# wvangansbeke/LaneDetection_End2End

Hardware: AMD Instinct MI355X
Metric: images/sec fwd+bwd, 256x512 2-lane bs32 (higher is better)
Workload: dtype f32; 1 GPU; BEV ERFNet + fused WLS fit + Area loss, 2 lanes, 256x512, batch 32 per GPU, fp32, train mode (BN batch stats, Dropout2d on), fwd+bwd, optimizer excluded; global_batch=32, parallelism=dp1, grad_allreduce=none

## Files before the change

lanedetection_end2end_amd/csrc/lf_conv.hip:

```cpp
#include <stdlib.h>
#include <string.h>

#include <atomic>
#include <map>
#include <mutex>
#include <tuple>
#include <utility>

#include <hip/hip_ext.h>

#include "lf_conv.h"
#include "lf_ldsdma.h"
#include "lf_types.h"

typedef float f32x4 __attribute__((ext_vector_type(4)));

namespace {

constexpr int MT = 4;
constexpr int WG_WAVES = 4;
constexpr int PIX_PER_WG = WG_WAVES * MT * 16;

__device__ __forceinline__ f32x4 ldg4(const float* p) { return *reinterpret_cast<const f32x4*>(p); }
typedef unsigned u32x4v __attribute__((vector_size(16)));
__device__ __forceinline__ __amdgpu_buffer_rsrc_t make_rsrc(const void* base, unsigned bytes) {
    return __builtin_amdgcn_make_buffer_rsrc(const_cast<void*>(base), 0, bytes, 0x00020000);
}
__device__ __forceinline__ f32x4 ldb4(__amdgpu_buffer_rsrc_t r, unsigned voff, unsigned soff) {
    return __builtin_bit_cast(f32x4, __builtin_amdgcn_raw_buffer_load_b128(r, (int)voff, (int)soff, 0));
}
__device__ __forceinline__ f32x4 zero4() { f32x4 z = {0.f, 0.f, 0.f, 0.f}; return z; }
typedef int i32x4 __attribute__((ext_vector_type(4)));
__device__ __forceinline__ f32x4 max0(f32x4 v) {
    i32x4 b = __builtin_bit_cast(i32x4, v);
    b.x = b.x > 0 ? b.x : 0; b.y = b.y > 0 ? b.y : 0; b.z = b.z > 0 ? b.z : 0; b.w = b.w > 0 ? b.w : 0;
    return __builtin_bit_cast(f32x4, b);
}
__device__ __forceinline__ f32x4 relu_keep_nan(f32x4 v) {
    v.x = v.x <= 0.f ? 0.f : v.x; v.y = v.y <= 0.f ? 0.f : v.y; v.z = v.z <= 0.f ? 0.f : v.z; v.w = v.w <= 0.f ? 0.f : v.w;
    return v;
}
__device__ __forceinline__ f32x4 keep_pos(f32x4 v, f32x4 m) {
    v.x = m.x > 0.f ? v.x : 0.f; v.y = m.y > 0.f ? v.y : 0.f; v.z = m.z > 0.f ? v.z : 0.f; v.w = m.w > 0.f ? v.w : 0.f;
    return v;
}
typedef unsigned u32x2v __attribute__((vector_size(8)));
template <bool S16>
__device__ __forceinline__ f32x4 epi_ld(__amdgpu_buffer_rsrc_t r, unsigned off, unsigned soff = 0u) {
    if constexpr (S16) {
        const u32x2v q = __builtin_amdgcn_raw_buffer_load_b64(r, (int)(off * 2u), (int)(soff * 2u), 0);
        f32x4 v;
        v.x = __uint_as_float(q[0] << 16); v.y = __uint_as_float(q[0] & 0xffff0000u);
        v.z = __uint_as_float(q[1] << 16); v.w = __uint_as_float(q[1] & 0xffff0000u);
        return v;
    } else return ldb4(r, off * 4u, soff * 4u);
}
template <bool S16>
__device__ __forceinline__ void epi_st(__amdgpu_buffer_rsrc_t r, unsigned off, f32x4 v) {
    if constexpr (S16) {
        lf_bf16x4 b;
        b[0] = (lf_bf16)v.x; b[1] = (lf_bf16)v.y; b[2] = (lf_bf16)v.z; b[3] = (lf_bf16)v.w;
        __builtin_amdgcn_raw_buffer_store_b64(__builtin_bit_cast(u32x2v, b), r, (int)(off * 2u), 0, 0);
    } else __builtin_amdgcn_raw_buffer_store_b128(__builtin_bit_cast(u32x4v, v), r, (int)(off * 4u), 0, 0);
}
__device__ __forceinline__ f32x4 round_bf16(f32x4 v) {
    v.x = (float)(lf_bf16)v.x; v.y = (float)(lf_bf16)v.y; v.z = (float)(lf_bf16)v.z; v.w = (float)(lf_bf16)v.w;
    return v;
}
typedef float f32x2 __attribute__((ext_vector_type(2)));
typedef __bf16 bf16x2 __attribute__((ext_vector_type(2)));
__device__ __forceinline__ unsigned split_pair(f32x2& v) {
    const unsigned u = __builtin_bit_cast(unsigned, __builtin_convertvector(v, bf16x2));
    v.x -= __uint_as_float(u << 16);
    v.y -= __uint_as_float(u & 0xffff0000u);
    return u;
}
template <int CTRL>
__device__ __forceinline__ float dpp_mov(float v) {
    return __builtin_bit_cast(float, __builtin_amdgcn_update_dpp(0, __builtin_bit_cast(int, v), CTRL, 0xf, 0xf, false));
}
__device__ __forceinline__ f32x4 bcast16(f32x4 v) {
    f32x4 r;
    r.x = dpp_mov<0x150>(v.x); r.y = dpp_mov<0x150>(v.y); r.z = dpp_mov<0x150>(v.z); r.w = dpp_mov<0x150>(v.w);
    return r;
}
__device__ __forceinline__ float sum16(float v) {
    v += dpp_mov<0xB1>(v);
    v += dpp_mov<0x4E>(v);
    v += dpp_mov<0x124>(v);
    v += dpp_mov<0x128>(v);
    return v;
}

#define LF_EPI_GROUPS 1
#define LF_EPI_ONE_TILE false
#define LF_EPI_TID threadIdx.x
#define LF_EPI_ROW1 false
#define LF_EPI_PIVOT true
#define LF_EPI_ACC(n, m) acc[n][m]
#define LF_EPI_FIRST(m) ((m) == 0)
#define LF_EPI_ROW_OK(tg) true
#define LF_EPI_HEAD \
      \
    const bool stats = (epi & (LF_EPI_STATS_SQ | LF_EPI_STATS_XHAT)) != 0; \
    constexpr bool NOBIAS = EPIC >= 0 && !(EPIC & LF_EPI_BIAS) && (EPIC & (LF_EPI_MASK | LF_EPI_ADD | LF_EPI_MASKBN | LF_EPI_STATS_XHAT)) != 0; \
    constexpr int NC = (NT % 2 == 0 && !LF_EPI_ONE_TILE) ? 2 : 1; \
     \
    constexpr bool HOISTM = HOISTV && !(EPIC >= 0 && (EPIC & LF_EPI_MASKBN) && (EPIC & LF_EPI_STATS_XHAT)); \
    const __amdgpu_buffer_rsrc_t r_dst = make_rsrc(a.dst, 0xffffffffu), r_add = make_rsrc(a.add_src, 0xffffffffu), \
                                 r_msk = make_rsrc(a.mask_src, 0xffffffffu), r_aux = make_rsrc(a.aux, 0xffffffffu), \
                                 r_bias = make_rsrc(a.bias, 0xffffffffu), r_msc = make_rsrc(a.msc, 0xffffffffu), \
                                 r_msh = make_rsrc(a.msh, 0xffffffffu), r_dm = make_rsrc(a.dm, 0xffffffffu); \
     \
    f32x4 s1[NT], s2[NT], bs[NOBIAS ? 1 : NT], hv[HOISTV ? NT : 1][2], piv[LF_EPI_PIVOT ? NT : 1]; \
_Pragma("unroll") \
    for (int n = 0; n < NT; ++n) { \
        const int co = cob + n * 16 + kq * 4; \
        s1[n] = zero4(); s2[n] = zero4(); piv[LF_EPI_PIVOT ? n : 0] = zero4(); \
        if constexpr (!NOBIAS) bs[n] = a.bias ? ldb4(r_bias, co * 4u, 0u) : zero4(); \
        if (HOISTV) { \
            if (HOISTM && (epi & LF_EPI_MASKBN)) { hv[n][0] = ldb4(r_msc, co * 4u, 0u); hv[n][1] = ldb4(r_msh, co * 4u, 0u); } \
        } \
    }
#define LF_EPI_TILE(m) \
    { \
        const unsigned dbase = (unsigned)(((pn[m] * g.Hd + pi[m] * g.dsh + g.dah) * g.Wd + pj[m] * g.dsw + g.daw) * g.d_pix + g.d_choff + cob + kq * 4); \
_Pragma("unroll") \
        for (int n0 = 0; n0 < NT; n0 += NC) { \
        f32x4 la[NC], lm[NC], lx[NC], ld[NC]; \
_Pragma("unroll") \
        for (int j = 0; j < NC; ++j) { \
            const int n = n0 + j; \
            if (epi & LF_EPI_ADD) la[j] = epi_ld<S16>(r_add, dbase + n * 16); \
            if (epi & LF_EPI_MASK) lm[j] = epi_ld<S16>(r_msk, dbase + n * 16); \
            if (epi & (LF_EPI_MASKBN | LF_EPI_STATS_XHAT)) lx[j] = epi_ld<S16>(r_aux, dbase + n * 16); \
            if ((epi & LF_EPI_STATS_XHAT) && a.dm && !LF_EPI_ROW1) ld[j] = ldb4(r_dm, (unsigned)(pn[m] * g.Cd + cob + n * 16 + kq * 4) * 4u, 0u); \
        } \
_Pragma("unroll") \
        for (int j = 0; j < NC; ++j) { \
            const int n = n0 + j; \
            f32x4 v = LF_EPI_ACC(n, m); \
            if constexpr (!NOBIAS) v += bs[n]; \
            if (epi & LF_EPI_ADD) v += la[j]; \
            if (epi & LF_EPI_MASK) v = keep_pos(v, lm[j]); \
            const int co = cob + n * 16 + kq * 4;    \
            if (epi & LF_EPI_MASKBN) v = keep_pos(v, lx[j] * (HOISTM ? hv[HOISTV ? n : 0][0] : ldb4(r_msc, co * 4u, 0u)) + (HOISTM ? hv[HOISTV ? n : 0][1] : ldb4(r_msh, co * 4u, 0u))); \
            if (epi & LF_EPI_RELU) v = S16 ? relu_keep_nan(v) : max0(v); \
            if (S16) v = round_bf16(v);    \
            if (pv[m]) epi_st<S16>(r_dst, dbase + n * 16, v); \
            if (!pv[m]) v = zero4(); \
            if (epi & LF_EPI_STATS_SQ) { \
                if (LF_EPI_PIVOT && LF_EPI_FIRST(m)) piv[LF_EPI_PIVOT ? n : 0] = bcast16(v); \
                f32x4 dv = LF_EPI_PIVOT ? v - piv[LF_EPI_PIVOT ? n : 0] : v; \
                if (!pv[m]) dv = zero4(); \
                s1[n] += dv; s2[n] += dv * dv; \
            } \
            if (epi & LF_EPI_STATS_XHAT) { \
                const f32x4 gm = (a.dm && !LF_EPI_ROW1) ? v * ld[j] : v; \
                s1[n] += gm; s2[n] += gm * lx[j];       \
            } \
        } \
        } \
    }
#define LF_EPI_TAIL \
    if (LF_EPI_ROW1 && (epi & LF_EPI_STATS_XHAT) && a.dm) { \
         \
_Pragma("unroll") \
        for (int n = 0; n < NT; ++n) { \
            const f32x4 dmv = ldb4(r_dm, (unsigned)(pn[0] * g.Cd + cob + n * 16 + kq * 4) * 4u, 0u); \
            s1[n] *= dmv; s2[n] *= dmv; \
        } \
    } \
    if (stats) { \
         \
        const int EW = wave & 3, EG = wave >> 2; \
        __shared__ float sred[LF_EPI_GROUPS][WG_WAVES][NT][4][8]; \
_Pragma("unroll") \
        for (int n = 0; n < NT; ++n) { \
            f32x4 r1, r2; \
            r1.x = sum16(s1[n].x); r1.y = sum16(s1[n].y); r1.z = sum16(s1[n].z); r1.w = sum16(s1[n].w); \
            r2.x = sum16(s2[n].x); r2.y = sum16(s2[n].y); r2.z = sum16(s2[n].z); r2.w = sum16(s2[n].w); \
            if (epi & LF_EPI_STATS_SQ) {       \
                const unsigned lf_t0 = (bx * (unsigned)(WG_WAVES * LF_EPI_GROUPS) + (unsigned)wave) * 64u; \
                const float nw = lf_t0 < npix ? (float)min(npix - lf_t0, 64u) : 0.f; \
                const float rn = nw > 0.f ? 1.f / nw : 0.f; \
                r2 = r2 - r1 * r1 * rn; \
                r2.x = fmaxf(r2.x, 0.f); r2.y = fmaxf(r2.y, 0.f); r2.z = fmaxf(r2.z, 0.f); r2.w = fmaxf(r2.w, 0.f); \
                if (LF_EPI_PIVOT) r1 = r1 + piv[LF_EPI_PIVOT ? n : 0] * nw; \
            } \
            if (pl == 0) { \
                float* d = sred[EG][EW][n][kq]; \
                d[0] = r1.x; d[1] = r1.y; d[2] = r1.z; d[3] = r1.w; d[4] = r2.x; d[5] = r2.y; d[6] = r2.z; d[7] = r2.w; \
            } \
        } \
        __syncthreads(); \
        if ((LF_EPI_TID & 255) < NT * 4 * 8 && LF_EPI_ROW_OK(LF_EPI_TID >> 8)) { \
            const int tg = LF_EPI_TID >> 8, tt = LF_EPI_TID & 255; \
            const int j = tt & 7, q = (tt >> 3) & 3, n = tt >> 5; \
            float v = sred[tg][0][n][q][j] + sred[tg][1][n][q][j] + sred[tg][2][n][q][j] + sred[tg][3][n][q][j]; \
            if ((epi & LF_EPI_STATS_SQ) && j >= 4) {       \
                const unsigned lf_tb = (bx * (unsigned)LF_EPI_GROUPS + (unsigned)tg) * (unsigned)(WG_WAVES * 64); \
                float nwv[4], sw[4], nt = 0.f, st = 0.f; \
_Pragma("unroll") \
                for (int w = 0; w < 4; ++w) { \
                    const unsigned t0w = lf_tb + (unsigned)w * 64u; \
                    nwv[w] = t0w < npix ? (float)min(npix - t0w, 64u) : 0.f; \
                    sw[w] = sred[tg][w][n][q][j - 4]; \
                    nt += nwv[w]; st += sw[w]; \
                } \
                const float mg = nt > 0.f ? st / nt : 0.f; \
_Pragma("unroll") \
                for (int w = 0; w < 4; ++w) \
                    if (nwv[w] > 0.f) { const float dmw = sw[w] / nwv[w] - mg; v += nwv[w] * dmw * dmw; } \
            } \
            const int co = cob + n * 16 + q * 4 + (j & 3); \
            a.stats[((long)(j >> 2) * g.Cd + co) * a.stats_ld + ((long)bx * LF_EPI_GROUPS + tg)] = v;       \
        } \
    }
#define LF_TAPGEMM_EPILOGUE \
    __builtin_amdgcn_s_setprio(3);    \
    LF_EPI_HEAD \
_Pragma("unroll") \
    for (int m = 0; m < MT; ++m) LF_EPI_TILE(m) \
    LF_EPI_TAIL

extern __shared__ __attribute__((aligned(16))) unsigned char lf_tap_lds[];
constexpr size_t LF_TAP_LDS_PER_TAP = (size_t)WG_WAVES * 64 * (sizeof(uint4) + sizeof(unsigned));

template <int NT, int PROC, int EPIC = -1, bool ROW1 = false, bool DBG = false>
__global__ __launch_bounds__(256, (EPIC >= 0 || NT < 4) ? 2 : 1) void tapgemm_kernel(const LfTapGeom g, const LfTapArgs a, const int pro, const int epi_rt) {
    const int epi = EPIC >= 0 ? EPIC : epi_rt;
    constexpr bool S16 = false, HOISTV = EPIC >= 0;
    unsigned long long tstamp[4] = {0ull, 0ull, 0ull, 0ull};
    if constexpr (DBG) tstamp[0] = __builtin_amdgcn_s_memrealtime();
    const unsigned npix = (unsigned)(g.N * g.Hl * g.Wl);
    const int cob = blockIdx.y * NT * 16;
    const unsigned ntiles = (npix + PIX_PER_WG - 1) / PIX_PER_WG;
    unsigned t_first = blockIdx.x, t_stride = gridDim.x, t_end = ntiles;
    if ((gridDim.x & 7u) == 0 && (ntiles & 7u) == 0) {
        const unsigned per = ntiles >> 3;
        t_first = (blockIdx.x & 7u) * per + (blockIdx.x >> 3); t_stride = gridDim.x >> 3; t_end = (blockIdx.x & 7u) * per + per;
    }
    for (unsigned bx = t_first; bx < t_end; bx += t_stride) {
    unsigned tid = threadIdx.x;
    asm volatile("" : "+v"(tid));
    const int lane = tid & 63, wave = tid >> 6;
    const int pl = lane & 15, kq = lane >> 4;
    const unsigned tile0 = (bx * WG_WAVES + (ROW1 ? __builtin_amdgcn_readfirstlane(wave) : wave)) * (MT * 16);

    int pn[MT], pi[MT], pj[MT];
    bool pv[MT];
    if constexpr (ROW1) {
        const unsigned q = tile0 < npix ? tile0 : 0u;
        const unsigned r = q / (unsigned)g.Wl;
        const int j0 = __builtin_amdgcn_readfirstlane((int)(q - r * (unsigned)g.Wl));
        const int n0 = __builtin_amdgcn_readfirstlane((int)(r / (unsigned)g.Hl));
        const int i0 = __builtin_amdgcn_readfirstlane((int)r) - n0 * g.Hl;
#pragma unroll
        for (int m = 0; m < MT; ++m) { pv[m] = tile0 < npix; pn[m] = n0; pi[m] = i0; pj[m] = j0 + m * 16 + pl; }
// ... 103 lines not shown
        if constexpr (DBG) tstamp[1] = __builtin_amdgcn_s_memrealtime();
        Step A, B;
        issue(A);
        finish(A);
        const int npairs = (nsteps + 1) >> 1;
        for (int pr = 0; pr < npairs; ++pr) {
            mma_restart(A);
            __builtin_amdgcn_sched_barrier(0);
            issue(B);
            __builtin_amdgcn_sched_barrier(0);
            mma(A, 1); mma(A, 2);
            __builtin_amdgcn_sched_barrier(0);
            finish(B);
            mma(A, 3);
            __builtin_amdgcn_sched_barrier(0);
            mma(B, 0);
            __builtin_amdgcn_sched_barrier(0);
            issue(A);
            __builtin_amdgcn_sched_barrier(0);
            mma(B, 1); mma(B, 2);
            __builtin_amdgcn_sched_barrier(0);
            finish(A);
            mma(B, 3);
            __builtin_amdgcn_sched_barrier(0);
        }
    }

#pragma unroll
    for (int n = 0; n < NT; ++n)
#pragma unroll
        for (int m = 0; m < MT; ++m) acc[n][m] += accl[n][m];
    if constexpr (!ROW1) {
        unsigned tid2 = threadIdx.x;
        asm volatile("" : "+v"(tid2));
        const unsigned tile0b = (bx * WG_WAVES + (tid2 >> 6)) * (MT * 16);
#pragma unroll
        for (int m = 0; m < MT; ++m) {
            const unsigned p = tile0b + m * 16 + (tid2 & 15u);
            pv[m] = p < npix;
            const unsigned q = pv[m] ? p : 0u;
            const unsigned r = q / (unsigned)g.Wl;
            pj[m] = (int)(q - r * (unsigned)g.Wl);
            pn[m] = (int)(r / (unsigned)g.Hl);
            pi[m] = (int)(r - (unsigned)pn[m] * (unsigned)g.Hl);
        }
    }
    if constexpr (DBG) {
        asm volatile("" ::"v"(acc[0][0][0]));
        tstamp[2] = __builtin_amdgcn_s_memrealtime();
    }
#undef LF_EPI_ONE_TILE
#define LF_EPI_ONE_TILE (!ROW1 && EPIC == (LF_EPI_ADD | LF_EPI_MASK | LF_EPI_STATS_XHAT))
#undef LF_EPI_TID
#define LF_EPI_TID tid
#undef LF_EPI_ROW1
#define LF_EPI_ROW1 ROW1
    LF_TAPGEMM_EPILOGUE
#undef LF_EPI_ONE_TILE
#define LF_EPI_ONE_TILE false
#undef LF_EPI_TID
#define LF_EPI_TID threadIdx.x
#undef LF_EPI_ROW1
#define LF_EPI_ROW1 false
    if (stats && bx + t_stride < t_end) __syncthreads();
    __builtin_amdgcn_s_setprio(0);
    }
    if constexpr (DBG) {
        asm volatile("s_waitcnt vmcnt(0)" ::: "memory");
        tstamp[3] = __builtin_amdgcn_s_memrealtime();
        const int lane = threadIdx.x & 63, wave = threadIdx.x >> 6;
        if (lane == 0 && a.dbg) {
            unsigned long long* d = a.dbg + ((unsigned long long)(blockIdx.y * gridDim.x + blockIdx.x) * WG_WAVES + wave) * 8;
            d[0] = tstamp[0]; d[1] = tstamp[1]; d[2] = tstamp[2]; d[3] = tstamp[3];
            unsigned hwid, xcc;
            asm volatile("s_getreg_b32 %0, hwreg(HW_REG_HW_ID)" : "=s"(hwid));
            asm volatile("s_getreg_b32 %0, hwreg(HW_REG_XCC_ID)" : "=s"(xcc));
            d[4] = (unsigned long long)hwid | ((unsigned long long)xcc << 32);
        }
    }
}

template <int CS, int PROC, int EPIC, int G>
__global__ __launch_bounds__(256 * G, G == 1 ? 2 : 1) void tapstream_kernel(const LfTapGeom g, const LfTapArgs a) {
    constexpr int NT = 4, NCG = CS / 16, NS = 3 * NCG, R = 8;
    constexpr int epi = EPIC;
    constexpr bool S16 = false, HOISTV = true;
    static_assert((4 * NS) % R == 0 && R <= NS && NS % 2 == 0, "ring positions and K-step pairs must be compile-time");
    const unsigned npix = (unsigned)(g.N * g.Hl * g.Wl);
    const int cob = blockIdx.y * 64;
    const unsigned ntiles = (npix + PIX_PER_WG - 1) / PIX_PER_WG, nunits = (ntiles + G - 1) / G;
    unsigned u_first = blockIdx.x, u_stride = gridDim.x, u_end = nunits;
    if ((gridDim.x & 7u) == 0 && (nunits & 7u) == 0) {
        const unsigned per = nunits >> 3;
        u_first = (blockIdx.x & 7u) * per + (blockIdx.x >> 3); u_stride = gridDim.x >> 3; u_end = (blockIdx.x & 7u) * per + per;
    }
    const int lane = threadIdx.x & 63, wave = threadIdx.x >> 6;
    const int pl = lane & 15, kq = lane >> 4;
    const unsigned wtile = (unsigned)__builtin_amdgcn_readfirstlane(wave);


    f32x4* const wl = reinterpret_cast<f32x4*>(lf_tap_lds);
    float* const pvec = reinterpret_cast<float*>(wl + NS * 256);
    struct WT { int n0, i0, j0; bool v; };
    auto coords = [&](unsigned u, bool live) -> WT {
        const unsigned tile0 = (u * (unsigned)(4 * G) + wtile) * 64u;
        WT c;
        c.v = live && tile0 < npix;
        const unsigned q = c.v ? tile0 : 0u;
        const unsigned r = q / (unsigned)g.Wl;
        c.j0 = __builtin_amdgcn_readfirstlane((int)(q - r * (unsigned)g.Wl));
        c.n0 = __builtin_amdgcn_readfirstlane((int)(r / (unsigned)g.Hl));
        c.i0 = __builtin_amdgcn_readfirstlane((int)r) - c.n0 * g.Hl;
        return c;
    };
    auto xoff = [&](const WT& c, int sub, int t, bool& in) -> unsigned {
        const int sy = c.i0 * g.ssh + g.tdh[t], sx = (c.j0 + sub * 16 + pl) * g.ssw + g.tdw[t];
        in = c.v && sy >= 0 && sy < g.Hs && sx >= 0 && sx < g.Ws;
        const int syc = min(max(sy, 0), g.Hs - 1), sxc = min(max(sx, 0), g.Ws - 1);
        const unsigned o = (unsigned)(((c.n0 * g.Hs + syc) * g.Ws + sxc) * g.s_pix + g.s_choff + kq * 4) * 4u;
        return (PROC == 0 && !in) ? LF_OOB : o;
    };
    const __amdgpu_buffer_rsrc_t rx = make_rsrc(a.src, (unsigned)min((long)g.N * g.Hs * g.Ws * g.s_pix * 4, (long)LF_OOB));
    auto xload = [&](const WT& c, int p) -> f32x4 {
        const int k = p % NS;
        bool in;
        const unsigned o = xoff(c, p / NS, k / NCG, in);
        return ldb4(rx, o, (unsigned)(k % NCG) * 64u);
    };

    f32x4 ring[R], wn[NT];
    WT cur = coords(u_first, u_first < u_end);
#pragma unroll
    for (int p = 0; p < R; ++p) ring[p] = xload(cur, p);
    {
        const __amdgpu_buffer_rsrc_t rw = make_rsrc(a.wp, (unsigned)(3 * CS * CS * 4));
        for (int idx = threadIdx.x; idx < NS * 256; idx += 256 * G) {
            const int col = idx & 63, row = idx >> 6;
            wl[((row >> 2) * 4 + (col >> 4)) * 64 + (row & 3) * 16 + (col & 15)] = ldb4(rw, (unsigned)(row * CS + cob + col) * 16u, 0u);
        }
        if constexpr (PROC == LF_PRO_BNRELU) {
            const __amdgpu_buffer_rsrc_t rsc = make_rsrc(a.pro_sc, CS * 4u), rsh = make_rsrc(a.pro_sh, CS * 4u);
            for (int i = threadIdx.x; i < 2 * CS; i += 256 * G)
                pvec[i] = __uint_as_float(__builtin_amdgcn_raw_buffer_load_b32(i < CS ? rsc : rsh, (i < CS ? i : i - CS) * 4, 0, 0));
        }
    }
    __syncthreads();
#pragma unroll
    for (int n = 0; n < NT; ++n) wn[n] = wl[n * 64 + lane];

#undef LF_EPI_GROUPS
#define LF_EPI_GROUPS G
#undef LF_EPI_ROW1
#define LF_EPI_ROW1 true
#undef LF_EPI_ACC
#define LF_EPI_ACC(n, m) acc[n]
#undef LF_EPI_FIRST
#define LF_EPI_FIRST(m) (sub == 0)
#undef LF_EPI_ROW_OK
#define LF_EPI_ROW_OK(tg) (bx * (unsigned)G + (unsigned)(tg) < ntiles)
    LF_EPI_HEAD
    for (unsigned bx = u_first; bx < u_end; bx += u_stride) {
        const WT nxt = coords(bx + u_stride, bx + u_stride < u_end);
        const int pn[1] = {cur.n0}, pi[1] = {cur.i0};
        const bool pv[1] = {cur.v};
#pragma unroll
        for (int sub = 0; sub < 4; ++sub) {
            f32x4 acc[NT], accl[NT];
#pragma unroll
            for (int k = 0; k < NS; ++k) {
                const int p = sub * NS + k, cg = k % NCG;
                f32x4 w[NT];
#pragma unroll
                for (int n = 0; n < NT; ++n) w[n] = wn[n];
#pragma unroll
                for (int n = 0; n < NT; ++n) wn[n] = wl[(((k + 1) % NS) * 4 + n) * 64 + lane];
                f32x4 x = ring[p % R];
                if constexpr (PROC == LF_PRO_BNRELU) {
                    bool in;
                    (void)xoff(cur, sub, k / NCG, in);
                    const f32x4 sc = *reinterpret_cast<const f32x4*>(pvec + cg * 16 + kq * 4);
                    const f32x4 sh = *reinterpret_cast<const f32x4*>(pvec + CS + cg * 16 + kq * 4);
                    f32x4 v = max0(x * sc + sh);
                    v.x = in ? v.x : 0.f; v.y = in ? v.y : 0.f; v.z = in ? v.z : 0.f; v.w = in ? v.w : 0.f;
                    x = v;
                }
                if (k % 2 == 0) {
#pragma unroll
                    for (int n = 0; n < NT; ++n) {
                        if (k == 0) accl[n] = zero4();
                        else { accl[n] += acc[n]; asm volatile("" : "+v"(accl[n])); }
                        acc[n] = __builtin_amdgcn_mfma_f32_16x16x4f32(w[n][0], x[0], zero4(), 0, 0, 0);
                    }
                }
#pragma unroll
                for (int s = (k % 2 == 0) ? 1 : 0; s < 4; ++s)
#pragma unroll
                    for (int n = 0; n < NT; ++n) acc[n] = __builtin_amdgcn_mfma_f32_16x16x4f32(w[n][s], x[s], acc[n], 0, 0, 0);
                if (p + R < 4 * NS) ring[p % R] = xload(cur, p + R);
                else ring[p % R] = xload(nxt, p + R - 4 * NS);
                __builtin_amdgcn_sched_barrier(0);
            }
#pragma unroll
            for (int n = 0; n < NT; ++n) acc[n] += accl[n];
            const int pj[1] = {cur.j0 + sub * 16 + pl};
            LF_EPI_TILE(0)
        }
        LF_EPI_TAIL
        if (stats) {
#pragma unroll
            for (int n = 0; n < NT; ++n) { s1[n] = zero4(); s2[n] = zero4(); }
            if (bx + u_stride < u_end) __syncthreads();
        }
        cur = nxt;
    }
#undef LF_EPI_GROUPS
#define LF_EPI_GROUPS 1
#undef LF_EPI_ROW1
#define LF_EPI_ROW1 false
#undef LF_EPI_ACC
#define LF_EPI_ACC(n, m) acc[n][m]
#undef LF_EPI_FIRST
#define LF_EPI_FIRST(m) ((m) == 0)
#undef LF_EPI_ROW_OK
#define LF_EPI_ROW_OK(tg) true
}

typedef __bf16 bf16x8 __attribute__((ext_vector_type(8)));
typedef unsigned u32x4 __attribute__((ext_vector_type(4)));

__device__ __forceinline__ bf16x8 cvt_bf16x8(f32x4 lo, f32x4 hi) {
    bf16x8 r;
    r[0] = (__bf16)lo.x; r[1] = (__bf16)lo.y; r[2] = (__bf16)lo.z; r[3] = (__bf16)lo.w;
    r[4] = (__bf16)hi.x; r[5] = (__bf16)hi.y; r[6] = (__bf16)hi.z; r[7] = (__bf16)hi.w;
    return r;
}

template <int NT, int PROC, int EPIC = -1, bool FAST = false>
__global__ __launch_bounds__(256, 2) void tapgemm_bf16_kernel(const LfTapGeom g, const LfTapArgs a, const int pro, const int epi_rt) {
    static_assert(!FAST || PROC == 0, "FAST: the out-of-range zero must be the operand itself");
    const int epi = EPIC >= 0 ? EPIC : epi_rt;
    constexpr bool HOISTV = true, S16 = true;
    const int lane = threadIdx.x & 63, wave = threadIdx.x >> 6;
    const int pl = lane & 15, kq = lane >> 4;
    const unsigned npix = (unsigned)(g.N * g.Hl * g.Wl);
    const int cob = blockIdx.y * NT * 16;
    unsigned bx = blockIdx.x;
    if ((gridDim.x & 7u) == 0) bx = (bx & 7u) * (gridDim.x >> 3) + (bx >> 3);
    const unsigned tile0 = (bx * WG_WAVES + wave) * (MT * 16);

    int pn[MT], pi[MT], pj[MT];
    bool pv[MT];
#pragma unroll
    for (int m = 0; m < MT; ++m) {
        const unsigned p = tile0 + m * 16 + pl;
        pv[m] = p < npix;
        const unsigned q = pv[m] ? p : 0u;
        const unsigned r = q / (unsigned)g.Wl;
        pj[m] = (int)(q - r * (unsigned)g.Wl);
        pn[m] = (int)(r / (unsigned)g.Hl);
        pi[m] = (int)(r - (unsigned)pn[m] * (unsigned)g.Hl);
    }
    f32x4 acc[NT][MT];
#pragma unroll
    for (int n = 0; n < NT; ++n)
#pragma unroll
        for (int m = 0; m < MT; ++m) acc[n][m] = zero4();

    struct Step { u32x4 w[NT]; f32x4 xl[MT]; f32x4 sc0, sc1, sh0, sh1; unsigned ok; };
    __shared__ uint4 tab_off[WG_WAVES][LF_MAX_TAPS][64];
    __shared__ unsigned tab_ok[WG_WAVES][LF_MAX_TAPS][64];
    const int ncb = (g.Cs + 31) >> 5;
    const int nsteps = g.ntaps * ncb;
    const bool part = FAST && (g.Cs & 31) != 0;
    const int nrows = part ? nsteps : g.ntaps;
    for (int r = 0; r < nrows; ++r) {
        const int t = part ? r / ncb : r, c0 = (part ? r - t * ncb : 0) * 32 + kq * 8;
        const int dh = g.tdh[t], dw = g.tdw[t];
        unsigned o[MT], okb = 0;
#pragma unroll
        for (int m = 0; m < MT; ++m) {
            const int sy = pi[m] * g.ssh + dh, sx = pj[m] * g.ssw + dw;
            const bool in = pv[m] && sy >= 0 && sy < g.Hs && sx >= 0 && sx < g.Ws;
            const int syc = min(max(sy, 0), g.Hs - 1), sxc = min(max(sx, 0), g.Ws - 1);
            o[m] = (unsigned)(((pn[m] * g.Hs + syc) * g.Ws + sxc) * g.s_pix + g.s_choff);
            if constexpr (FAST) o[m] = (in && c0 < g.Cs) ? (o[m] + c0) * 2u : LF_OOB;
            okb |= (in ? 1u : 0u) << m;
        }
        tab_off[wave][r][lane] = make_uint4(o[0], o[1], o[2], o[3]);
        tab_ok[wave][r][lane] = okb;
    }
    const __amdgpu_buffer_rsrc_t rw = make_rsrc(a.wp16, 0xffffffffu),
                                 rx = make_rsrc(a.src, FAST ? (unsigned)min((long)g.N * g.Hs * g.Ws * g.s_pix * 2, (long)LF_OOB) : 0xffffffffu),
                                 rsc = make_rsrc(a.pro_sc, 0xffffffffu), rsh = make_rsrc(a.pro_sh, 0xffffffffu);
    const unsigned wlane = (unsigned)(kq * g.Cd + cob + pl) * 16u;
    const int wstep = g.Cd * 32;
    const int ntaps = g.ntaps;
    const int wlast = (nsteps - 1) * wstep;
// ... 1314 lines not shown
    const long npix = (long)g.N * g.Hl * g.Wl;
    return lf_cdiv(npix, PIX_PER_WG);
}
int lf_tapgemm_stat_rows_for(const LfTapGeom& g, const LfTapArgs& a) {
    (void)a;
    return lf_cdiv((long)g.N * g.Hl * g.Wl, PIX_PER_WG);
}

namespace {
std::mutex g_launch_state_mutex;
int current_device() {
    int dev = 0;
    return hipGetDevice(&dev) == hipSuccess ? dev : -1;
}
template <typename K>
int resident_workgroups(K kernel, size_t lds, int block = 256) {
    static std::map<std::tuple<int, const void*, size_t>, int> cache;
    const int dev = current_device();
    const std::tuple<int, const void*, size_t> key(dev, reinterpret_cast<const void*>(kernel), lds);
    std::lock_guard<std::mutex> lock(g_launch_state_mutex);
    auto it = cache.find(key);
    if (it != cache.end()) return it->second;
    int cus = 0, nb = 0;
    if (dev < 0 || hipDeviceGetAttribute(&cus, hipDeviceAttributeMultiprocessorCount, dev) != hipSuccess ||
        hipOccupancyMaxActiveBlocksPerMultiprocessor(&nb, kernel, block, lds) != hipSuccess || nb < 1 || cus < 1)
        return cache[key] = 1 << 30;
    return cache[key] = nb * cus;
}
bool allow_big_lds(const void* kernel, int bytes) {
    static std::map<std::pair<int, const void*>, bool> done;
    const std::pair<int, const void*> key(current_device(), kernel);
    std::lock_guard<std::mutex> lock(g_launch_state_mutex);
    auto it = done.find(key);
    if (it != done.end()) return it->second;
    return done[key] = hipFuncSetAttribute(kernel, hipFuncAttributeMaxDynamicSharedMemorySize, bytes) == hipSuccess;
}
thread_local unsigned g_launch_flags = 0;
template <typename K>
void launch_tapgemm(K kernel, dim3 grid, size_t lds, hipStream_t st, const LfTapGeom& g, const LfTapArgs& a, int pro, int epi) {
    const unsigned res = (unsigned)resident_workgroups(kernel, lds) / grid.y;
    if (grid.x > res && res >= 8) grid.x = res & ~7u;
    if (g_launch_flags) hipExtLaunchKernelGGL(kernel, grid, dim3(256), (unsigned)lds, st, nullptr, nullptr, g_launch_flags, g, a, pro, epi);
    else hipLaunchKernelGGL(kernel, grid, dim3(256), lds, st, g, a, pro, epi);
}
template <int EPIV, bool DBGV = false>
void launch_bf16_ring(unsigned nitems, hipStream_t st, const LfTapGeom& g, const LfTapArgs& a, int pro, int epi) {
    auto kern = tapgemm_bf16_ring_kernel<EPIV, DBGV>;
    const size_t ring_lds = (size_t)LB_STAGES * LB_STAGE_BYTES;
    unsigned gx = nitems;
    const unsigned res = (unsigned)resident_workgroups(kern, ring_lds);
    if (gx > res && res >= 8) gx = res & ~7u;
    hipLaunchKernelGGL(kern, dim3(gx), dim3(256), ring_lds, st, g, a, pro, epi);
}
template <int CBV, int EPIV, int PROV = 0>
bool launch_bf16_wl(unsigned nitems, hipStream_t st, const LfTapGeom& g, const LfTapArgs& a, int pro, int epi) {
    auto kern = tapgemm_bf16_wl_kernel<CBV, EPIV, PROV>;
    const size_t lds = WlCfg<CBV, EPIV, PROV>::LDS;
    if (!allow_big_lds(reinterpret_cast<const void*>(kern), 160 * 1024 - 4096)) return false;
    unsigned gx = nitems;
    const unsigned res = (unsigned)resident_workgroups(kern, lds);
    if (gx > res && res >= 8) gx = res & ~7u;
    hipLaunchKernelGGL(kern, dim3(gx), dim3(256), lds, st, g, a, pro, epi);
    return true;
}
template <int EPIV>
bool launch_bf16_wv(unsigned ntiles, hipStream_t st, const LfTapGeom& g, const LfTapArgs& a, int pro, int epi) {
    auto kern = tapgemm_bf16_wv_kernel<EPIV>;
    const size_t lds = WvCfg<EPIV>::LDS;
    if (!allow_big_lds(reinterpret_cast<const void*>(kern), 160 * 1024 - 4096)) return false;
    unsigned gx = ntiles;
    const unsigned res = (unsigned)resident_workgroups(kern, lds);
    if (gx > res && res >= 8) gx = res & ~7u;
    hipLaunchKernelGGL(kern, dim3(gx), dim3(256), lds, st, g, a, pro, epi);
    return true;
}
std::atomic<int> g_stream_mode{1}, g_stream_cap{0};
enum { LF_STREAM_RELU = 1, LF_STREAM_STATS = 2, LF_STREAM_MASK = 4, LF_STREAM_PRO = 8, LF_STREAM_X48 = 16, LF_STREAM_X38 = 32 };
constexpr int g_stream_routed[2] = {LF_STREAM_RELU | LF_STREAM_STATS | LF_STREAM_MASK | LF_STREAM_PRO | LF_STREAM_X48 | LF_STREAM_X38,
                                    0};
template <int CS, int PROV, int EPIV>
bool launch_tapstream(hipStream_t st, const LfTapGeom& g, const LfTapArgs& a) {
    constexpr int G = CS == 128 ? 2 : 1;
    auto kern = tapstream_kernel<CS, PROV, EPIV, G>;
    const size_t lds = (size_t)3 * (CS / 16) * 4096 + (PROV == LF_PRO_BNRELU ? 2 * CS * sizeof(float) : 0);
    if (!allow_big_lds(reinterpret_cast<const void*>(kern), 160 * 1024 - 4096)) return false;
    const unsigned ntiles = (unsigned)lf_cdiv((long)g.N * g.Hl * g.Wl, PIX_PER_WG);
    dim3 grid((ntiles + G - 1) / G, CS / 64);
    const unsigned res = (unsigned)resident_workgroups(kern, lds, 256 * G) / grid.y;
    if (grid.x > res && res >= 8) grid.x = res & ~7u;
    const unsigned cap = (unsigned)g_stream_cap.load();
    if (cap > 0 && grid.x > cap) grid.x = cap;
    if (g_launch_flags) hipExtLaunchKernelGGL(kern, grid, dim3(256 * G), (unsigned)lds, st, nullptr, nullptr, g_launch_flags, g, a);
    else hipLaunchKernelGGL(kern, grid, dim3(256 * G), lds, st, g, a);
    return true;
}
template <int CS>
bool route_tapstream(int variant, hipStream_t st, const LfTapGeom& g, const LfTapArgs& a) {
    switch (variant) {
        case LF_STREAM_RELU: return launch_tapstream<CS, 0, LF_EPI_RELU>(st, g, a);
        case LF_STREAM_STATS: return launch_tapstream<CS, 0, LF_EPI_STATS_SQ>(st, g, a);
        case LF_STREAM_MASK: return launch_tapstream<CS, 0, LF_EPI_MASK>(st, g, a);
        case LF_STREAM_PRO: return launch_tapstream<CS, 1, LF_EPI_RELU>(st, g, a);
        case LF_STREAM_X48: if constexpr (CS == 64) return launch_tapstream<CS, 0, LF_EPI_MASKBN | LF_EPI_STATS_XHAT>(st, g, a); else return false;
        case LF_STREAM_X38: if constexpr (CS == 64) return launch_tapstream<CS, 0, LF_EPI_ADD | LF_EPI_MASK | LF_EPI_STATS_XHAT>(st, g, a); else return false;
        default: return false;
    }
}
}

void lf_tapgemm_set_fp32_stream(int mode, int max_workgroups) { g_stream_mode = mode; g_stream_cap = max_workgroups > 0 ? max_workgroups : 0; }

int lf_tapgemm_launch_unordered(const LfTapGeom& g, const LfTapArgs& a, int pro, int epi, hipStream_t st) {
    g_launch_flags = hipExtAnyOrderLaunch;
    const int rc = lf_tapgemm_launch(g, a, pro, epi, st);
    g_launch_flags = 0;
    return rc;
}

int lf_tapgemm_launch(const LfTapGeom& g, const LfTapArgs& a, int pro, int epi, hipStream_t st) {
    LF_REQUIRE(g.Cs % 16 == 0 && g.Cd % 16 == 0, "tapgemm: channels must be multiples of 16 (Cs=%d Cd=%d)", g.Cs, g.Cd);
    LF_REQUIRE(g.s_pix % 4 == 0 && g.s_choff % 4 == 0 && g.d_pix % 4 == 0 && g.d_choff % 4 == 0, "tapgemm: unaligned channel layout");
    LF_REQUIRE(g.ntaps >= 1 && g.ntaps <= LF_MAX_TAPS, "tapgemm: bad tap count %d", g.ntaps);
    const long npix = (long)g.N * g.Hl * g.Wl;
    LF_REQUIRE(npix < (1L << 30), "tapgemm: too many pixels (%ld)", npix);
    const int nt = pick_nt(g.Cd);
    dim3 grid(lf_cdiv(npix, PIX_PER_WG), g.Cd / (16 * nt));
    LF_REQUIRE((long)g.N * g.Hs * g.Ws * g.s_pix * 4 < (long)LF_OOB, "tapgemm: source tensor too large for 32-bit byte offsets");
    LF_REQUIRE((long)g.N * g.Hd * g.Wd * g.d_pix * 4 < (long)LF_OOB, "tapgemm: destination tensor too large for 32-bit byte offsets");
#define LF_TG(NTV)                                                                                                       \
    do {                                                                                                                 \
        if (pro == LF_PRO_BNRELU) launch_tapgemm(tapgemm_kernel<NTV, 1>, grid, tap_lds, st, g, a, pro, epi);  \
        else launch_tapgemm(tapgemm_kernel<NTV, 0>, grid, tap_lds, st, g, a, pro, epi);                       \
    } while (0)
#define LF_TG4(PROV, EPIV)                                                                                               \
    do {                                                                                                                 \
        if ((g.Wl & 63) == 0) launch_tapgemm(tapgemm_kernel<4, PROV, EPIV, true>, grid, tap_lds, st, g, a, pro, epi);  \
        else launch_tapgemm(tapgemm_kernel<4, PROV, EPIV, false>, grid, tap_lds, st, g, a, pro, epi);    \
    } while (0)
    const size_t tap_lds = LF_TAP_LDS_PER_TAP * g.ntaps;
    constexpr int BRES = LF_EPI_ADD | LF_EPI_RELU | LF_EPI_BIAS;
    const int epis = (epi == (LF_EPI_ADD | LF_EPI_RELU) && a.bias) ? BRES
                   : ((epi & (LF_EPI_MASK | LF_EPI_ADD | LF_EPI_MASKBN | LF_EPI_STATS_XHAT)) && a.bias) ? -2 : epi;
    LF_REQUIRE(!a.s16 || a.wp16, "tapgemm: bf16 tensors need the bf16 matrix-core kernel (wp16)");
    if (a.split && a.wp48 && !a.wp16 && lf_tapgemm_split_ok(g)) {
        LF_REQUIRE(a.split == 9, "tapgemm: split must be 9 (got %d; the 6-term form was removed in round 6)", a.split);
        LfTapArgs b = a;
        b.wp16 = a.wp48;
        const dim3 grid2((unsigned)(npix / (2 * PIX_PER_WG)), g.Cd / 64);
        if (a.dbg) {
            LF_REQUIRE(pro == LF_PRO_NONE && epi == 0, "tapgemm: phase stamps are compiled into the plain convolution only");
            hipLaunchKernelGGL((tapgemm_split_kernel<4, 0, 0, true>), grid2, dim3(512), 0, st, g, b, pro, epi);
        } else {
#define LF_TS9(PROV, EPIV) hipLaunchKernelGGL((tapgemm_split_kernel<4, PROV, EPIV>), grid2, dim3(512), 0, st, g, b, pro, epi)
            if (pro == LF_PRO_BNRELU && epi == LF_EPI_RELU) LF_TS9(1, LF_EPI_RELU);
            else if (pro == LF_PRO_BNRELU) LF_TS9(1, -1);
            else switch (epis) {
                case 0: LF_TS9(0, 0); break;
                case LF_EPI_RELU: LF_TS9(0, LF_EPI_RELU); break;
                case LF_EPI_MASK: LF_TS9(0, LF_EPI_MASK); break;
                case LF_EPI_ADD: LF_TS9(0, LF_EPI_ADD); break;
                case LF_EPI_STATS_SQ: LF_TS9(0, LF_EPI_STATS_SQ); break;
                case LF_EPI_MASK | LF_EPI_STATS_XHAT: LF_TS9(0, LF_EPI_MASK | LF_EPI_STATS_XHAT); break;
                case LF_EPI_ADD | LF_EPI_MASK | LF_EPI_STATS_XHAT: LF_TS9(0, LF_EPI_ADD | LF_EPI_MASK | LF_EPI_STATS_XHAT); break;
                case LF_EPI_MASKBN | LF_EPI_STATS_XHAT: LF_TS9(0, LF_EPI_MASKBN | LF_EPI_STATS_XHAT); break;
                default: LF_TS9(0, -1); break;
            }
#undef LF_TS9
// ... 1325 lines not shown
```

Before: 2019 images/sec.

## Software-pipeline tapstream epilogue into next sub-tile's MFMA loop

For CS=64 single-group tapstream kernels with epilogue loads (mask/maskbn/xhat, no add), the epilogue of the previous sub-tile is split into load and apply phases that are interleaved at fixed K-steps of the next sub-tile's MFMA loop, hiding epilogue memory latency behind compute. The stats reduction uses double-buffered shared memory to drop a per-tile __syncthreads, and MASKBN scale/shift vectors are staged in LDS when combined with XHAT stats. The ring depth is reduced for MASKBN variants to free registers. This raises register pressure and adds complexity in tile retirement ordering.

Result: no change. 2031 images/sec (median of 6 runs) (+0.6%).

```diff
diff --git a/lanedetection_end2end_amd/csrc/lf_conv.hip b/lanedetection_end2end_amd/csrc/lf_conv.hip
--- a/lanedetection_end2end_amd/csrc/lf_conv.hip
+++ b/lanedetection_end2end_amd/csrc/lf_conv.hip
@@ -100,6 +100,10 @@
 #define LF_EPI_ACC(n, m) acc[n][m]
 #define LF_EPI_FIRST(m) ((m) == 0)
 #define LF_EPI_ROW_OK(tg) true
+#define LF_EPI_MSC(co) ldb4(r_msc, (co) * 4u, 0u)
+#define LF_EPI_MSH(co) ldb4(r_msh, (co) * 4u, 0u)
+#define LF_EPI_SRED_COPIES 1
+#define LF_EPI_SRED_COPY 0
 #define LF_EPI_HEAD \
       \
     const bool stats = (epi & (LF_EPI_STATS_SQ | LF_EPI_STATS_XHAT)) != 0; \
@@ -122,29 +126,26 @@
             if (HOISTM && (epi & LF_EPI_MASKBN)) { hv[n][0] = ldb4(r_msc, co * 4u, 0u); hv[n][1] = ldb4(r_msh, co * 4u, 0u); } \
         } \
     }
-#define LF_EPI_TILE(m) \
-    { \
-        const unsigned dbase = (unsigned)(((pn[m] * g.Hd + pi[m] * g.dsh + g.dah) * g.Wd + pj[m] * g.dsw + g.daw) * g.d_pix + g.d_choff + cob + kq * 4); \
-_Pragma("unroll") \
-        for (int n0 = 0; n0 < NT; n0 += NC) { \
-        f32x4 la[NC], lm[NC], lx[NC], ld[NC]; \
+#define LF_EPI_DBASE(m) ((unsigned)(((pn[m] * g.Hd + pi[m] * g.dsh + g.dah) * g.Wd + pj[m] * g.dsw + g.daw) * g.d_pix + g.d_choff + cob + kq * 4))
+#define LF_EPI_LOAD(m, n0, B) \
 _Pragma("unroll") \
         for (int j = 0; j < NC; ++j) { \
-            const int n = n0 + j; \
-            if (epi & LF_EPI_ADD) la[j] = epi_ld<S16>(r_add, dbase + n * 16); \
-            if (epi & LF_EPI_MASK) lm[j] = epi_ld<S16>(r_msk, dbase + n * 16); \
-            if (epi & (LF_EPI_MASKBN | LF_EPI_STATS_XHAT)) lx[j] = epi_ld<S16>(r_aux, dbase + n * 16); \
-            if ((epi & LF_EPI_STATS_XHAT) && a.dm && !LF_EPI_ROW1) ld[j] = ldb4(r_dm, (unsigned)(pn[m] * g.Cd + cob + n * 16 + kq * 4) * 4u, 0u); \
-        } \
+            const int n = (n0) + j; \
+            if (epi & LF_EPI_ADD) la[(B) + j] = epi_ld<S16>(r_add, dbase + n * 16); \
+            if (epi & LF_EPI_MASK) lm[(B) + j] = epi_ld<S16>(r_msk, dbase + n * 16); \
+            if (epi & (LF_EPI_MASKBN | LF_EPI_STATS_XHAT)) lx[(B) + j] = epi_ld<S16>(r_aux, dbase + n * 16); \
+            if ((epi & LF_EPI_STATS_XHAT) && a.dm && !LF_EPI_ROW1) ld[(B) + j] = ldb4(r_dm, (unsigned)(pn[m] * g.Cd + cob + n * 16 + kq * 4) * 4u, 0u); \
+        }
+#define LF_EPI_APPLY(m, n0, B) \
 _Pragma("unroll") \
         for (int j = 0; j < NC; ++j) { \
-            const int n = n0 + j; \
+            const int n = (n0) + j; \
             f32x4 v = LF_EPI_ACC(n, m); \
             if constexpr (!NOBIAS) v += bs[n]; \
-            if (epi & LF_EPI_ADD) v += la[j]; \
-            if (epi & LF_EPI_MASK) v = keep_pos(v, lm[j]); \
+            if (epi & LF_EPI_ADD) v += la[(B) + j]; \
+            if (epi & LF_EPI_MASK) v = keep_pos(v, lm[(B) + j]); \
             const int co = cob + n * 16 + kq * 4;    \
-            if (epi & LF_EPI_MASKBN) v = keep_pos(v, lx[j] * (HOISTM ? hv[HOISTV ? n : 0][0] : ldb4(r_msc, co * 4u, 0u)) + (HOISTM ? hv[HOISTV ? n : 0][1] : ldb4(r_msh, co * 4u, 0u))); \
+            if (epi & LF_EPI_MASKBN) v = keep_pos(v, lx[(B) + j] * (HOISTM ? hv[HOISTV ? n : 0][0] : LF_EPI_MSC(co)) + (HOISTM ? hv[HOISTV ? n : 0][1] : LF_EPI_MSH(co))); \
             if (epi & LF_EPI_RELU) v = S16 ? relu_keep_nan(v) : max0(v); \
             if (S16) v = round_bf16(v);    \
             if (pv[m]) epi_st<S16>(r_dst, dbase + n * 16, v); \
@@ -156,10 +157,18 @@
                 s1[n] += dv; s2[n] += dv * dv; \
             } \
             if (epi & LF_EPI_STATS_XHAT) { \
-                const f32x4 gm = (a.dm && !LF_EPI_ROW1) ? v * ld[j] : v; \
-                s1[n] += gm; s2[n] += gm * lx[j];       \
+                const f32x4 gm = (a.dm && !LF_EPI_ROW1) ? v * ld[(B) + j] : v; \
+                s1[n] += gm; s2[n] += gm * lx[(B) + j];       \
             } \
-        } \
+        }
+#define LF_EPI_TILE(m) \
+    { \
+        const unsigned dbase = LF_EPI_DBASE(m); \
+_Pragma("unroll") \
+        for (int n0 = 0; n0 < NT; n0 += NC) { \
+        f32x4 la[NC], lm[NC], lx[NC], ld[NC]; \
+        LF_EPI_LOAD(m, n0, 0) \
+        LF_EPI_APPLY(m, n0, 0) \
         } \
     }
 #define LF_EPI_TAIL \
@@ -174,7 +183,8 @@
     if (stats) { \
          \
         const int EW = wave & 3, EG = wave >> 2; \
-        __shared__ float sred[LF_EPI_GROUPS][WG_WAVES][NT][4][8]; \
+        __shared__ float sred_all[LF_EPI_SRED_COPIES][LF_EPI_GROUPS][WG_WAVES][NT][4][8]; \
+        float (*const sred)[WG_WAVES][NT][4][8] = sred_all[LF_EPI_SRED_COPY]; \
 _Pragma("unroll") \
         for (int n = 0; n < NT; ++n) { \
             f32x4 r1, r2; \
@@ -444,7 +454,10 @@
 
 template <int CS, int PROC, int EPIC, int G>
 __global__ __launch_bounds__(256 * G, G == 1 ? 2 : 1) void tapstream_kernel(const LfTapGeom g, const LfTapArgs a) {
-    constexpr int NT = 4, NCG = CS / 16, NS = 3 * NCG, R = 8;
+    constexpr int NT = 4, NCG = CS / 16, NS = 3 * NCG;
+    constexpr bool EPI_LOADS = EPIC >= 0 && (EPIC & (LF_EPI_ADD | LF_EPI_MASK | LF_EPI_MASKBN | LF_EPI_STATS_XHAT)) != 0;
+    constexpr bool PIPE = CS == 64 && G == 1 && PROC == 0 && EPIC >= 0 && EPI_LOADS && !(EPIC & LF_EPI_ADD);
+    constexpr int R = (PIPE && (EPIC & LF_EPI_MASKBN) != 0) ? 4 : 8;
     constexpr int epi = EPIC;
     constexpr bool S16 = false, HOISTV = true;
     static_assert((4 * NS) % R == 0 && R <= NS && NS % 2 == 0, "ring positions and K-step pairs must be compile-time");
@@ -463,6 +476,9 @@
 
     f32x4* const wl = reinterpret_cast<f32x4*>(lf_tap_lds);
     float* const pvec = reinterpret_cast<float*>(wl + NS * 256);
+    constexpr bool MVEC_LDS = EPIC >= 0 && (EPIC & LF_EPI_MASKBN) != 0 && (EPIC & LF_EPI_STATS_XHAT) != 0;
+    float* const mvec = pvec + (PROC == LF_PRO_BNRELU ? 2 * CS : 0);
+    (void)mvec;
     struct WT { int n0, i0, j0; bool v; };
     auto coords = [&](unsigned u, bool live) -> WT {
         const unsigned tile0 = (u * (unsigned)(4 * G) + wtile) * 64u;
@@ -505,6 +521,11 @@
             for (int i = threadIdx.x; i < 2 * CS; i += 256 * G)
                 pvec[i] = __uint_as_float(__builtin_amdgcn_raw_buffer_load_b32(i < CS ? rsc : rsh, (i < CS ? i : i - CS) * 4, 0, 0));
         }
+        if constexpr (MVEC_LDS) {
+            const __amdgpu_buffer_rsrc_t rmc = make_rsrc(a.msc, (unsigned)g.Cd * 4u), rmh = make_rsrc(a.msh, (unsigned)g.Cd * 4u);
+            for (int i = threadIdx.x; i < 128; i += 256 * G)
+                mvec[i] = __uint_as_float(__builtin_amdgcn_raw_buffer_load_b32(i < 64 ? rmc : rmh, (cob + (i & 63)) * 4, 0, 0));
+        }
     }
     __syncthreads();
 #pragma unroll
@@ -515,19 +536,52 @@
 #undef LF_EPI_ROW1
 #define LF_EPI_ROW1 true
 #undef LF_EPI_ACC
-#define LF_EPI_ACC(n, m) acc[n]
+#define LF_EPI_ACC(n, m) fin[n]
 #undef LF_EPI_FIRST
-#define LF_EPI_FIRST(m) (sub == 0)
+#define LF_EPI_FIRST(m) (esub == 0)
 #undef LF_EPI_ROW_OK
 #define LF_EPI_ROW_OK(tg) (bx * (unsigned)G + (unsigned)(tg) < ntiles)
+#undef LF_EPI_MSC
+#define LF_EPI_MSC(co) (MVEC_LDS ? *reinterpret_cast<const f32x4*>(mvec + ((co) - cob)) : ldb4(r_msc, (co) * 4u, 0u))
+#undef LF_EPI_MSH
+#define LF_EPI_MSH(co) (MVEC_LDS ? *reinterpret_cast<const f32x4*>(mvec + 64 + ((co) - cob)) : ldb4(r_msh, (co) * 4u, 0u))
+#undef LF_EPI_SRED_COPIES
+#define LF_EPI_SRED_COPIES (G == 1 ? 2 : 1)
+#undef LF_EPI_SRED_COPY
+#define LF_EPI_SRED_COPY (G == 1 ? par : 0u)
+#define LF_STREAM_EPI_SCOPE(T, U, S) \
+    const int esub = (S); \
+    const unsigned bx = (U); \
+    const int pn[1] = {(T).n0}, pi[1] = {(T).i0}, pj[1] = {(T).j0 + esub * 16 + pl}; \
+    const bool pv[1] = {(T).v}; \
+    (void)esub; (void)bx; (void)pn; (void)pi; (void)pj; (void)pv;
     LF_EPI_HEAD
-    for (unsigned bx = u_first; bx < u_end; bx += u_stride) {
-        const WT nxt = coords(bx + u_stride, bx + u_stride < u_end);
-        const int pn[1] = {cur.n0}, pi[1] = {cur.i0};
-        const bool pv[1] = {cur.v};
+    constexpr int LD0 = 0, LD1 = 1, AP0 = 8, AP1 = 10;
+    static_assert(AP0 < NS && AP1 < NS && LD0 <= AP0 && LD1 <= AP1 && AP0 < AP1, "the retiring sub-tile must be done before fin is overwritten");
+    f32x4 fin[NT], la[NT], lm[NT], lx[NT], ld[NT];
+    WT prv = cur;
+    unsigned pbx = u_first, par = 0;
+    bool pend = false;
+    auto tile_tail = [&](const WT& t, unsigned u) {
+        LF_STREAM_EPI_SCOPE(t, u, 3)
+        LF_EPI_TAIL
+        if (stats) {
+#pragma unroll
+            for (int n = 0; n < NT; ++n) { s1[n] = zero4(); s2[n] = zero4(); }
+            if (G != 1 && u + u_stride < u_end) __syncthreads();
+        }
+        par ^= 1u;
+    };
+    (void)prv; (void)pbx; (void)pend; (void)la; (void)lm; (void)lx; (void)ld;
+    for (unsigned ubx = u_first; ubx < u_end; ubx += u_stride) {
+        const WT nxt = coords(ubx + u_stride, ubx + u_stride < u_end);
 #pragma unroll
         for (int sub = 0; sub < 4; ++sub) {
             f32x4 acc[NT], accl[NT];
+            const WT& ret = sub == 0 ? prv : cur;
+            const unsigned rbx = sub == 0 ? pbx : ubx;
+            const bool retire = PIPE && (sub > 0 || pend);
+            (void)ret; (void)rbx; (void)retire;
 #pragma unroll
             for (int k = 0; k < NS; ++k) {
                 const int p = sub * NS + k, cg = k % NCG;
@@ -558,23 +612,55 @@
                 for (int s = (k % 2 == 0) ? 1 : 0; s < 4; ++s)
 #pragma unroll
                     for (int n = 0; n < NT; ++n) acc[n] = __builtin_amdgcn_mfma_f32_16x16x4f32(w[n][s], x[s], acc[n], 0, 0, 0);
+                if constexpr (PIPE) {
+                    if (retire && (k == LD0 || k == LD1 || k == AP0 || k == AP1)) {
+                        LF_STREAM_EPI_SCOPE(ret, rbx, (sub + 3) & 3)
+                        const unsigned dbase = LF_EPI_DBASE(0);
+                        if (k == AP0) { LF_EPI_APPLY(0, 0, 0) }
+                        if (k == AP1) { LF_EPI_APPLY(0, NC, NC) }
+                        if (k == LD0 && EPI_LOADS) { LF_EPI_LOAD(0, 0, 0) }
+                        if (k == LD1 && EPI_LOADS) { LF_EPI_LOAD(0, NC, NC) }
+                    }
+                }
                 if (p + R < 4 * NS) ring[p % R] = xload(cur, p + R);
                 else ring[p % R] = xload(nxt, p + R - 4 * NS);
                 __builtin_amdgcn_sched_barrier(0);
             }
-#pragma unroll
-            for (int n = 0; n < NT; ++n) acc[n] += accl[n];
-            const int pj[1] = {cur.j0 + sub * 16 + pl};
-            LF_EPI_TILE(0)
-        }
-        LF_EPI_TAIL
-        if (stats) {
-#pragma unroll
-            for (int n = 0; n < NT; ++n) { s1[n] = zero4(); s2[n] = zero4(); }
-            if (bx + u_stride < u_end) __syncthreads();
+            if constexpr (PIPE) {
+                if (sub == 0 && pend) tile_tail(prv, pbx);
+#pragma unroll
+                for (int n = 0; n < NT; ++n) { fin[n] = acc[n] + accl[n]; asm volatile("" : "+v"(fin[n])); }
+            } else {
+#pragma unroll
+                for (int n = 0; n < NT; ++n) fin[n] = acc[n] + accl[n];
+                LF_STREAM_EPI_SCOPE(cur, ubx, sub)
+                LF_EPI_TILE(0)
+            }
+        }
+        if constexpr (PIPE) { prv = cur; pbx = ubx; pend = true; }
+        else {
+            tile_tail(cur, ubx);
         }
         cur = nxt;
     }
+    if constexpr (PIPE) {
+        if (pend) {
+            {
+                LF_STREAM_EPI_SCOPE(prv, pbx, 3)
+                LF_EPI_TILE(0)
+            }
+            tile_tail(prv, pbx);
+        }
+    }
+#undef LF_STREAM_EPI_SCOPE
+#undef LF_EPI_MSC
+#define LF_EPI_MSC(co) ldb4(r_msc, (co) * 4u, 0u)
+#undef LF_EPI_MSH
+#define LF_EPI_MSH(co) ldb4(r_msh, (co) * 4u, 0u)
+#undef LF_EPI_SRED_COPIES
+#define LF_EPI_SRED_COPIES 1
+#undef LF_EPI_SRED_COPY
+#define LF_EPI_SRED_COPY 0
 #undef LF_EPI_GROUPS
 #define LF_EPI_GROUPS 1
 #undef LF_EPI_ROW1
@@ -2055,7 +2141,8 @@
 bool launch_tapstream(hipStream_t st, const LfTapGeom& g, const LfTapArgs& a) {
     constexpr int G = CS == 128 ? 2 : 1;
     auto kern = tapstream_kernel<CS, PROV, EPIV, G>;
-    const size_t lds = (size_t)3 * (CS / 16) * 4096 + (PROV == LF_PRO_BNRELU ? 2 * CS * sizeof(float) : 0);
+    const size_t lds = (size_t)3 * (CS / 16) * 4096 + (PROV == LF_PRO_BNRELU ? 2 * CS * sizeof(float) : 0) +
+                       ((EPIV & LF_EPI_MASKBN) && (EPIV & LF_EPI_STATS_XHAT) ? 128 * sizeof(float) : 0);
     if (!allow_big_lds(reinterpret_cast<const void*>(kern), 160 * 1024 - 4096)) return false;
     const unsigned ntiles = (unsigned)lf_cdiv((long)g.N * g.Hl * g.Wl, PIX_PER_WG);
     dim3 grid((ntiles + G - 1) / G, CS / 64);
```
